# jgrss/cultionet

Measured on AMD Instinct MI355X. Metric: train_chips_per_sec, higher is better.
Workload: dtype f32

## Files before the change

cultionet_amd/_lib.py:

```python
from __future__ import annotations

import ctypes
import os
from ctypes import c_double, c_float, c_int, c_long, c_ulonglong, c_void_p

_HERE = os.path.dirname(os.path.abspath(__file__))
LIB_PATH = os.environ.get("CN_LIB_PATH") or os.path.join(_HERE, "csrc", "libcultionet_hip.so")

P = c_void_p
I, L, F, U64 = c_int, c_long, c_float, c_ulonglong

SIGNATURES = {
    "cn_version": [],
    "cn_conv_kpad": [I],
    "cn_conv_npad": [I],
    "cn_pack_weights_f32": [P, P, I, I, I, L, L, L, P],
    "cn_pack_weights_batched_f32": [P, I, P],
    "cn_conv2d_fwd_f32": [P, L, P, P, P, L, I, I, I, I, I, I, I, I, I, I, I, P],
    "cn_conv2d_bwd_data_f32": [P, L, P, P, L, I, I, I, I, I, I, I, I, I, I, I, P],
    "cn_conv2d_bwd_weight_f32": [P, L, P, L, P, I, I, I, I, I, I, I, I, I, I, P, L, P],
    "cn_conv_set_workspace": [P, P, L],
    "cn_conv_set_autotune": [I],
    "cn_conv2d_fwd_grouped_f32": [I, P, L, P, P, P, L, I, I, I, I, I, I, I, I, P, P, I, P],
    "cn_conv2d_bwd_data_grouped_f32": [I, P, L, P, P, L, I, I, I, I, I, P, P, I, P, P, I, P],
    "cn_conv2d_bwd_weight_grouped_f32": [I, P, L, P, L, P, I, I, I, I, I, I, I, I, I, I, P, L, P],
    "cn_thin_conv3x3_fwd_f32": [P, L, P, P, P, L, I, I, I, I, I, I, I, I, P, P],
    "cn_thin_conv3x3_bwd_data_f32": [P, L, P, P, L, I, I, I, I, I, I, I, I, I, P, P],
    "cn_thin_conv3x3_bwd_weight_f32": [P, L, P, L, P, I, I, I, I, I, I, I, I, P],
    "cn_conv_transpose2d_fwd_f32": [P, L, P, P, P, L, I, I, I, I, I, I, I, I, I, I, I, P],
    "cn_conv_transpose2d_bwd_data_f32": [P, L, P, P, L, I, I, I, I, I, I, I, I, I, I, I, P],
    "cn_conv_transpose2d_bwd_weight_f32": [P, L, P, L, P, I, I, I, I, I, I, I, I, I, I, P, L, P],
    "cn_channel_sum_f32": [P, L, I, I, I, P, I, P],
    "cn_bn_workspace_doubles": [I],
    "cn_bn_act_fwd_f32": [P, L, P, P, P, P, P, L, P, L, P, P, P, I, I, I, I, F, F, I, P],
    "cn_bn_act_bwd_f32": [P, L, P, L, P, P, P, P, P, L, P, P, P, P, I, I, I, I, I, I, I, P],
    "cn_bn_act_group_fwd_f32": [I, P, L, P, P, P, P, P, L, P, L, P, P, P, I, I, I, I, F, F, I, I, P],
    "cn_bn_act_group_bwd_f32": [I, P, L, P, L, P, P, P, P, P, L, P, P, P, P, I, I, I, I, I, I, P],
    "cn_layernorm_c_fwd_f32": [P, L, P, P, P, L, P, L, P, P, I, I, I, F, P],
    "cn_layernorm_c_workspace_floats": [I, I, I],
    "cn_layernorm_c_bwd_f32": [P, L, P, L, P, P, P, P, L, P, P, I, I, I, I, P, L, P],
    "cn_sca_pool_fwd_f32": [P, L, I, I, I, P, P, P, P, P, P],
    "cn_sca_pool_bwd_f32": [P, P, P, P, P, P, L, I, I, I, I, P],
    "cn_sca_mlp_fwd_f32": [P, P, P, P, P, P, P, P, P, I, I, I, P],
    "cn_sca_mlp_bwd_f32": [P, P, P, P, P, P, P, P, P, P, P, P, P, P, P, P, I, I, I, P],
    "cn_sca_apply_fwd_f32": [P, L, P, P, P, P, L, I, I, I, P],
    "cn_sca_apply_bwd_f32": [P, L, P, L, P, P, P, P, L, I, P, P, P, P, I, I, I, P],
    "cn_na2d_fwd_f32": [P, L, P, L, P, I, I, I, I, I, I, I, F, U64, P, P],
    "cn_na2d_bwd_f32": [P, L, P, L, P, P, P, L, I, I, I, I, I, I, I, F, U64, P, P],
    "cn_convt_taps_fwd_f32": [P, L, P, P, L, I, I, I, I, I, I, I, I, I, P],
    "cn_convt_taps_bwd_f32": [P, L, P, L, I, I, I, I, I, I, I, I, I, P],
    "cn_bilinear_fwd_f32": [P, L, P, L, I, I, I, I, I, I, I, I, P],
    "cn_bilinear_bwd_f32": [P, L, P, L, I, I, I, I, I, I, I, I, I, P],
    "cn_copy_f32": [P, L, P, L, I, L, I, P],
    "cn_add_f32": [P, L, P, L, P, L, I, L, P],
    "cn_fill_f32": [P, L, F, P],
    "cn_dropout_f32": [P, L, P, L, I, I, I, F, U64, P, I, I, P],
    "cn_rng_advance_u64": [P, U64, I, P],
    "cn_adaptive_maxpool_fwd_f32": [P, L, P, L, P, I, I, I, I, I, I, P],
    "cn_adaptive_maxpool_bwd_f32": [P, L, P, P, L, I, I, I, I, I, I, I, P],
    "cn_final_combine_fwd_f32": [P, P, P, P, P, P, P, I, I, F, P],
    "cn_final_combine_bwd_f32": [P, P, P, P, P, P, P, P, P, P, P, P, P, P, I, I, F, P],
    "cn_tanimoto_fwd_f32": [P, L, P, P, P, I, I, I, I, I, L, I, F, I, P, P, P, F, P, P],
    "cn_tanimoto_bwd_f32": [P, L, P, P, P, I, I, I, I, I, L, P, F, P, L, I, P],
    "cn_tanimoto_multi_fwd_f32": [I, P, I, L, I, F, I, P, P, P, P, P],
    "cn_tanimoto_multi_bwd_f32": [I, P, I, L, P, P],
    "cn_eval_metrics_f32": [P, P, P, P, P, I, F, L, P, P, P, P],
    "cn_grad_sumsq_f32": [P, L, P, P],
    "cn_adamw_step_f32": [P, P, P, P, L, F, F, F, F, F, I, F, P, F, P],
    "cn_grad_sumsq_seg_f32": [P, L, P, I, I, P, P],
    "cn_adamw_step_seg_f32": [P, P, P, P, L, P, I, I, I, F, F, F, F, F, F, P, F, P],
    "cn_pack_timeconv_f32": [P, P, I, I, I, I, I, P],
    "cn_fold_timeconv_grad_f32": [P, P, I, I, I, I, P],
    "cn_prepare_chips_f32": [P, I, P, P, P, I, I, L, F, F, F, P],
    "cn_predictions_to_u16": [P, P, P, P, I, I, I, I, I, I, I, F, P],
    "cn_bconv_packed_elems": [I, I, I],
# ... 116 lines not shown
```

cultionet_amd/csrc/cn_conv.hip:

```cpp
#include "cn_common.h"
#include "cn_conv_geom.h"
#include "cn_profile.h"

#include <cstdlib>

#define KC 8

static int cn_reduce_slices(const CnConvGeom& g, hipStream_t stream);

template <int TN, int TM>
__device__ __forceinline__ void cn_igemm_epilogue(const CnConvGeom& g, const f32x16 (&acc)[TN][TM],
                                                  const bool (&pix_ok)[TM], const int (&out_off)[TM], int co_base,
                                                  int half, int grp, int split, int b,
                                                  const float* __restrict__ bias, float* __restrict__ y) {
  const int HWout = g.Hout * g.Wout;
  const bool sliced = g.slice_stride != 0;
  float* yb = sliced ? g.part + (long)(grp * g.splits + split) * g.slice_stride + (long)b * g.Cout * HWout
                     : y + (long)b * g.ybs;
  const bool first = split == 0;
#pragma unroll
  for (int tn = 0; tn < TN; ++tn) {
#pragma unroll
    for (int r = 0; r < 16; ++r) {
      const int co = co_base + tn * 32 + (r & 3) + 8 * (r >> 2) + 4 * half;
      if (co < g.Cout) {
        const float bv = (bias != nullptr && first) ? bias[co] : 0.f;
#pragma unroll
        for (int tm = 0; tm < TM; ++tm) {
          if (pix_ok[tm]) {
            float* dst = yb + (long)co * HWout + out_off[tm];
            const float v = acc[tn][tm][r] + bv;
            if (sliced) {
              *dst = acc[tn][tm][r];
            } else if (g.atomic_out) {
              atomicAdd(dst, v);
            } else if (g.accumulate) {
              *dst += v;
            } else {
              *dst = v;
            }
          }
        }
      }
    }
  }
}

template <int WAVES_N, int TN, int NI_T>
__global__ __launch_bounds__(256) void cn_conv_igemm_kernel(const CnConvGeom g) {
  constexpr int WAVES_M = 4 / WAVES_N;
  constexpr int MT = WAVES_M * 64;
  constexpr int NT = WAVES_N * TN * 32;
  constexpr int WI = (CN_MAX_TAPS * KC * (NT / 4) + 255) / 256;
  extern __shared__ __attribute__((aligned(16))) float smem[];
  float* in_lds = smem;
  float* w_lds = smem + g.w_lds_off;
// ... 542 lines not shown
}

struct CnPlan {
  int total_tiles, max_plane, max_vplane, max_taps;
  int max_rplane, max_absdx;
  double flops;
};

static CnPlan cn_plan(CnConvGeom& g, int MT) {
  CnPlan p = {0, 0, 0, 0, 0, 0, 0.0};
  for (int c = 0; c < g.ncls; ++c) {
    CnConvClass& k = g.cls[c];
    const int Mimg = k.Hg * k.Wg;
    int rows_g = (MT + k.Wg - 2) / k.Wg + 1;
    if (rows_g > k.Hg) rows_g = k.Hg;
    k.min_dy = 0; k.min_dx = 0;
    int max_dy = 0, max_dx = 0;
    for (int t = 0; t < k.ntaps; ++t) {
      if (t == 0 || k.dy[t] < k.min_dy) k.min_dy = k.dy[t];
      if (t == 0 || k.dx[t] < k.min_dx) k.min_dx = k.dx[t];
      if (t == 0 || k.dy[t] > max_dy) max_dy = k.dy[t];
      if (t == 0 || k.dx[t] > max_dx) max_dx = k.dx[t];
    }
    const int rows = (rows_g - 1) * g.is + (max_dy - k.min_dy) + 1;
    k.pitch = (k.Wg - 1) * g.is + (max_dx - k.min_dx) + 1;
    k.plane = rows * k.pitch;
    k.vplane = (rows * g.Win + (max_dx - k.min_dx) + 4 + 3) / 4 * 4;
    k.rows = rows;
    {
      const int rpitch = (g.Win + 3) / 4 * 4 + 4;
      if ((rows + 1) * rpitch + 4 > p.max_rplane) p.max_rplane = (rows + 1) * rpitch + 4;
    }
    if (-k.min_dx > p.max_absdx) p.max_absdx = -k.min_dx;
    if (max_dx > p.max_absdx) p.max_absdx = max_dx;
    k.tiles_per_img = (Mimg + MT - 1) / MT;
    k.block_begin = p.total_tiles;
    p.total_tiles += g.B * k.tiles_per_img;
    if (k.plane > p.max_plane) p.max_plane = k.plane;
    if (k.vplane > p.max_vplane) p.max_vplane = k.vplane;
    if (k.ntaps > p.max_taps) p.max_taps = k.ntaps;
    p.flops += 2.0 * g.B * Mimg * (double)g.Cout * g.Cin * k.ntaps;
  }
  g.interleave = 0;
  if (g.ncls > 1 && g.want_interleave) {
    bool same = true;
    for (int c = 1; c < g.ncls; ++c) same = same && g.cls[c].tiles_per_img == g.cls[0].tiles_per_img;
    g.interleave = same ? 1 : 0;
  }
  return p;
}

struct CnChoice { int cfg, splits, cps; double cost; };

static double cn_launch_cost(long blocks, int cps, double mt_units, int splits, double out_elems) {
  const double F = 273.0, R = 170.0;
  const double c1 = 36.7 + 0.614 * mt_units, c2 = 30.0 + 1.19 * mt_units;
  const long full = blocks / 512, rem = blocks % 512;
  double c = full * (F + cps * c2);
  if (rem > 0) c += F + cps * (rem > 256 ? c2 : c1);
  if (splits > 1) c += R + out_elems * 4.0 * (2.0 * splits + 1.0) / 8.0e6 * (128.0 / 7.5);
  return c;
}

static thread_local float* g_conv_ws;
static thread_local long g_conv_ws_floats;

static CnChoice cn_choose(const CnConvGeom& g0, const int* mts, int ncfg, int NT, bool allow_split) {
  const int nchunks = (g0.Cin + KC - 1) / KC;
  const int ny = (g0.Cout + NT - 1) / NT;
  const int G = g0.G > 0 ? g0.G : 1;
  const double out_elems = (double)g0.B * g0.Cout * g0.Hout * g0.Wout * (g0.shared_y ? 1 : G);
  CnChoice best = {0, 1, nchunks > 0 ? nchunks : 1, 1e300};
  int forced = 0;
  {
    static const char* dbg = getenv("CN_DBG_SPLITS");
    if (dbg) forced = atoi(dbg) < 1 ? 1 : atoi(dbg);
  }
  long ws_cap = 32;
  if (g_conv_ws != nullptr) {
    const long stride = ((long)g0.B * g0.Cout * g0.Hout * g0.Wout + 3) / 4 * 4;
    ws_cap = g_conv_ws_floats / (stride * G);
  }
  int forced_cfg = -1;
  {
    static const char* dbgc = getenv("CN_DBG_CFG");
    if (dbgc) forced_cfg = atoi(dbgc);
  }
  for (int i = 0; i < ncfg; ++i) {
    if (forced_cfg >= 0 && i != (forced_cfg < ncfg ? forced_cfg : ncfg - 1)) continue;
    CnConvGeom gi = g0;
    const CnPlan p = cn_plan(gi, mts[i]);
    if (p.total_tiles <= 0) continue;
    const long base = (long)p.total_tiles * ny;
    int max_splits = (allow_split && p.max_taps > 0 && nchunks >= 4) ? nchunks / 2 : 1;
    if (max_splits > 32) max_splits = 32;
    if (max_splits > ws_cap) max_splits = ws_cap < 1 ? 1 : (int)ws_cap;
    const double taps = p.total_tiles > 0 ? p.flops / (2.0 * g0.Cout * g0.Cin * (double)mts[i] * p.total_tiles) : 9.0;
    const double chunk_units = (double)mts[i] * NT / 128.0 * (taps < 9.0 ? taps : 9.0) / 9.0;
    for (int sp = 1; sp <= max_splits; ++sp) {
      if (forced && sp != (forced > max_splits ? max_splits : forced)) continue;
      const int cps = (nchunks + sp - 1) / sp;
      const int splits = (nchunks + cps - 1) / cps;
      if (splits != sp && !forced) continue;
      const double cost = cn_launch_cost(base * splits, cps, chunk_units, splits, out_elems);
      if (cost < best.cost * (i == best.cfg ? 1.0 : 0.98)) best = {i, splits, cps, cost};
    }
  }
  return best;
}


#include <mutex>
#include <unordered_map>
namespace {
struct CnWs { float* p; long n; };
std::mutex g_ws_mu;
std::unordered_map<void*, CnWs> g_ws_by_stream;
}

extern "C" int cn_conv_set_workspace(void* stream, float* ws, long ws_floats) {
  if (ws != nullptr && ((reinterpret_cast<uintptr_t>(ws) & 15) || ws_floats < 0)) return CN_ERR_ARG;
  std::lock_guard<std::mutex> lk(g_ws_mu);
  if (ws == nullptr) g_ws_by_stream.erase(stream);
  else g_ws_by_stream[stream] = {ws, ws_floats};
  return CN_OK;
}

static void cn_bind_ws(void* stream) {
  std::lock_guard<std::mutex> lk(g_ws_mu);
  auto it = g_ws_by_stream.find(stream);
  if (it == g_ws_by_stream.end()) { g_conv_ws = nullptr; g_conv_ws_floats = 0; }
  else { g_conv_ws = it->second.p; g_conv_ws_floats = it->second.n; }
}

struct CnReduceArgs {
  const float* part;
  long slice_stride;
  int nsum;
  int ngrp;
  float* y[CN_MAX_GROUPS];
  const float* bias[CN_MAX_GROUPS * CN_MAX_GROUPS];
  int nbias;
  long ybs;
  int B, Cout, HW, accumulate;
};

__global__ __launch_bounds__(256) void cn_conv_reduce_kernel(const CnReduceArgs a) {
  const long n = (long)a.Cout * a.HW;
  const int b = blockIdx.y, gi = blockIdx.z;
  const float* p0 = a.part + (long)gi * a.nsum * a.slice_stride + (long)b * n;
  float* yb = a.y[gi] + (long)b * a.ybs;
  for (long i = (blockIdx.x * 256L + threadIdx.x) * 4; i < n; i += (long)gridDim.x * 1024) {
    if (i + 3 < n && (n & 3) == 0 && (a.ybs & 3) == 0 && (reinterpret_cast<uintptr_t>(yb) & 15) == 0) {
      f32x4 s = *reinterpret_cast<const f32x4*>(p0 + i);
      for (int k = 1; k < a.nsum; ++k) s += *reinterpret_cast<const f32x4*>(p0 + (long)k * a.slice_stride + i);
#pragma unroll
      for (int e = 0; e < 4; ++e) {
        const int c = (int)((i + e) / a.HW);
// ... 168 lines not shown
    __syncthreads();
#pragma unroll
    for (int k = 0; k < NA; ++k) *reinterpret_cast<f32x4*>(a_lds + (tid + k * 256) * 4) = ra[k];
#pragma unroll
    for (int k = 0; k < NB; ++k)
      if (tid + k * 256 < KC1 * MT / 4) *reinterpret_cast<f32x4*>(b_lds + (tid + k * 256) * 4) = rb[k];
    __syncthreads();
    if (ch + 1 < nchunks) CN_G1_PREFETCH((ch + 1) * KC1);
    const float* ap = a_lds + half * NT + wn * 32 + l31;
    const float* bp = b_lds + half * MT + l31;
#pragma unroll
    for (int k2 = 0; k2 < KC1 / 2; ++k2) {
      const float av = ap[k2 * 2 * NT];
#pragma unroll
      for (int tm = 0; tm < TM; ++tm)
        acc[tm] = __builtin_amdgcn_mfma_f32_32x32x2f32(av, bp[k2 * 2 * MT + tm * 32], acc[tm], 0, 0, 0);
    }
  }
#undef CN_G1_PREFETCH
  float* yb = y + (long)b * g.ybs;
#pragma unroll
  for (int r = 0; r < 16; ++r) {
    const int co = n0 + wn * 32 + (r & 3) + 8 * (r >> 2) + 4 * half;
    if (co < g.Cout) {
      const float bv = bias != nullptr ? bias[co] : 0.f;
#pragma unroll
      for (int tm = 0; tm < TM; ++tm) {
        const int p = p0 + tm * 32 + l31;
        if (p < g.HW) {
          float* dst = yb + (long)co * g.HW + p;
          const float v = acc[tm][r] + bv;
          *dst = g.accumulate ? *dst + v : v;
        }
      }
    }
  }
}

static int cn_conv1x1_launch(const float* x, long xbs, const float* wp, const float* bias, float* y, long ybs, int B,
                             int Cin, int HW, int Cout, int accumulate, hipStream_t stream) {
  if ((HW & 3) || (xbs & 3) || (reinterpret_cast<uintptr_t>(x) & 15)) return CN_ERR_ARG;
  CnGemm1x1 g = {};
  g.B = B; g.Cin = Cin; g.Cout = Cout; g.HW = HW; g.xbs = xbs; g.ybs = ybs; g.accumulate = accumulate;
  g.Kpad = cn_conv_kpad(Cin);
  g.Npad = cn_conv_npad(Cout);
  if (cn_pick_nt(Cout) != 128) return CN_ERR_ARG;
  g.grid_y = (Cout + 127) / 128;
  const long t160 = (long)B * ((HW + 159) / 160) * g.grid_y, t128 = (long)B * ((HW + 127) / 128) * g.grid_y;
  const bool use160 = ((t160 + 511) / 512) * 160 <= ((t128 + 511) / 512) * 128;
  const long blocks = use160 ? t160 : t128;
  if (blocks < 256) return CN_ERR_ARG;
  g.tiles_per_img = use160 ? (HW + 159) / 160 : (HW + 127) / 128;
  g.grid_x = B * g.tiles_per_img;
  const double flops = 2.0 * B * HW * (double)Cout * Cin;
  cn_prof_name("cn_conv1x1_kernel<%d>", use160 ? 5 : 4);
  cn_prof_desc("gemm1x1<%d> B%d %d->%d HW%d grid%dx%d", use160 ? 5 : 4, B, Cin, Cout, HW, g.grid_x, g.grid_y);
  cn_prof_before(stream);
  if (use160)
    CN_LAUNCH((cn_conv1x1_kernel<5>), dim3(cn_xcd_grid(blocks)), dim3(256), 0, stream, x, wp, bias, y, g);
  else
    CN_LAUNCH((cn_conv1x1_kernel<4>), dim3(cn_xcd_grid(blocks)), dim3(256), 0, stream, x, wp, bias, y, g);
  cn_prof_after(stream, 0, flops);
  return cn_check_launch();
}

#include <functional>
static int g_autotune = 0;
static std::unordered_map<uint64_t, CnChoice> g_tuned;
static std::mutex g_tune_mu;

extern "C" int cn_conv_set_autotune(int on) {
  std::lock_guard<std::mutex> lk(g_tune_mu);
  g_autotune = on ? 1 : 0;
  if (!on) g_tuned.clear();
  return CN_OK;
}

static uint64_t cn_tune_key(const CnConvGeom& g, bool vec, int nt, bool allow_split) {
  uint64_t h = 1469598103934665603ull;
  auto mix = [&](long v) { h = (h ^ (uint64_t)v) * 1099511628211ull; };
  mix(g.B); mix(g.Cin); mix(g.Hin); mix(g.Win); mix(g.Cout); mix(g.Hout); mix(g.Wout); mix(g.is); mix(g.os);
  mix(g.ncls); mix(g.G); mix(g.shared_y); mix(vec); mix(nt); mix(allow_split); mix(g_conv_ws != nullptr);
  for (int c = 0; c < g.ncls; ++c) {
    const CnConvClass& k = g.cls[c];
    mix(k.Hg); mix(k.Wg); mix(k.ntaps); mix(k.grp);
    for (int t = 0; t < k.ntaps; ++t) { mix(k.dy[t]); mix(k.dx[t]); }
  }
  return h;
}

static CnChoice cn_autotune(const CnConvGeom& g, const int* mts, int ncfg, int nt, bool allow_split,
                            const CnChoice& model, const std::function<int(const CnChoice&, CnConvGeom&)>& run,
                            hipStream_t stream) {
  static const int split_set[] = {1, 2, 3, 4, 6, 8, 12, 16, 24, 32};
  const int nchunks = (g.Cin + KC - 1) / KC;
  const int ny = (g.Cout + nt - 1) / nt;
  long ws_cap = 32;
  if (g_conv_ws != nullptr) {
    const long stride = ((long)g.B * g.Cout * g.Hout * g.Wout + 3) / 4 * 4;
    ws_cap = g_conv_ws_floats / (stride * (g.G > 0 ? g.G : 1));
  }
  hipEvent_t e0, e1;
  if (hipEventCreate(&e0) != hipSuccess || hipEventCreate(&e1) != hipSuccess) return model;
  CnChoice best = model;
  float best_ms = 1e30f;
  for (int i = 0; i < ncfg; ++i) {
    CnConvGeom gi = g;
    const CnPlan p = cn_plan(gi, mts[i]);
    if (p.total_tiles <= 0) continue;
    int max_splits = (allow_split && p.max_taps > 0 && nchunks >= 4) ? nchunks / 2 : 1;
    if (max_splits > 32) max_splits = 32;
    if (max_splits > ws_cap) max_splits = ws_cap < 1 ? 1 : (int)ws_cap;
    for (int sp : split_set) {
      if (sp > max_splits) break;
      const int cps = (nchunks + sp - 1) / sp;
      const int splits = (nchunks + cps - 1) / cps;
      if (splits != sp) continue;
      if ((long)p.total_tiles * ny * splits > 8192) continue;
      const CnChoice c = {i, splits, cps, 0.0};
      float ms = 0.f;
      bool ok = true;
      for (int rep = 0; rep < 2 && ok; ++rep) {
        CnConvGeom gg = g;
        ok = hipEventRecord(e0, stream) == hipSuccess && run(c, gg) == CN_OK &&
             hipEventRecord(e1, stream) == hipSuccess && hipEventSynchronize(e1) == hipSuccess &&
             hipEventElapsedTime(&ms, e0, e1) == hipSuccess;
      }
      if (ok && ms < best_ms) { best_ms = ms; best = c; }
    }
  }
  (void)hipEventDestroy(e0);
  (void)hipEventDestroy(e1);
  return best;
}

int cn_conv_igemm_launch(CnConvGeom& g, hipStream_t stream) {
  if (g.ncls < 1 || g.ncls > CN_MAX_CLASSES || g.B <= 0 || g.G < 1) return g.B <= 0 ? CN_OK : CN_ERR_ARG;
  g.splits = 1;
  const float* x = g.gx[0]; const float* wp = g.gwp[0]; const float* bias = g.gbias[0]; float* y = g.gy[0];
  g.Kpad = cn_conv_kpad(g.Cin);
  g.Npad = cn_conv_npad(g.Cout);
  const int nt = cn_pick_nt(g.Cout);
  const bool dense_out = g.ybs == (long)g.Cout * g.Hout * g.Wout;
  const bool ws_fits = g_conv_ws != nullptr &&
                       (((long)g.B * g.Cout * g.Hout * g.Wout + 3) / 4 * 4) * g.G * 32 <= g_conv_ws_floats;
  const bool allow_split = dense_out || g.accumulate || ws_fits;
  if (g.G > 1 && g.shared_y && !allow_split) return CN_ERR_ARG;
  const int hw4 = (int)(((long)g.Hin * g.Win) % 4);
  g.odd_planes = (hw4 == 1 && !(g.is > 1 && (long)g.Hin * g.Win > 4096)) ? 1 : 0;
  bool vec = (hw4 == 0 || g.odd_planes) && (g.xbs % 4 == 0);
  if (g.is > 1 && (long)g.Hin * g.Win > 4096) vec = false;
  if ((long)g.Cin * g.Hin * g.Win * 4 >= (1L << 31) || (long)CN_MAX_TAPS * cn_conv_kpad(g.Cin) * g.Npad * 4 >= (1L << 31))
    return CN_ERR_ARG;
  for (int i = 0; i < g.G; ++i) vec = vec && ((reinterpret_cast<uintptr_t>(g.gx[i]) & 15) == 0);
  if (vec) {
    CnConvGeom t = g;
    vec = cn_plan(t, 256).max_vplane <= 4 * 1024;
  }
  static const int mts128[3] = {128, 96, 160};
  static const int mts128d[1] = {128};
  static const int mts256[1] = {256};
  const int* mts = nt == 128 ? (vec ? mts128 : mts128d) : mts256;
  const int ncfg = (nt == 128 && vec) ? 3 : 1;
  auto run = [&](const CnChoice& c, CnConvGeom& gg) -> int {
    if (nt == 128) {
      if (vec) {
        switch (c.cfg) {
          case 1: return cn_launch_vec_cfg<4, 1, 3>(x, wp, bias, y, gg, c.splits, c.cps, stream);
          case 2: return cn_launch_vec_cfg<4, 1, 5>(x, wp, bias, y, gg, c.splits, c.cps, stream);
          default: return cn_launch_vec_cfg<2, 2, 2>(x, wp, bias, y, gg, c.splits, c.cps, stream);
        }
      }
      return cn_launch_dword_cfg<2, 2>(x, wp, bias, y, gg, c.splits, c.cps, stream);
    }
    int rc;
    if (nt == 64) {
      if (vec) return cn_launch_vec_cfg<1, 2, 2>(x, wp, bias, y, gg, c.splits, c.cps, stream);
      rc = cn_launch_dword_cfg<1, 2>(x, wp, bias, y, gg, c.splits, c.cps, stream);
    } else {
      if (vec) return cn_launch_vec_cfg<1, 1, 2>(x, wp, bias, y, gg, c.splits, c.cps, stream);
      rc = cn_launch_dword_cfg<1, 1>(x, wp, bias, y, gg, c.splits, c.cps, stream);
    }
    if (rc == CN_ERR_LDS) {
      CnConvGeom g2 = gg;
      rc = cn_launch_dword_cfg<2, 2>(x, wp, bias, y, g2, c.splits, c.cps, stream);
    }
    return rc;
  };
  CnChoice c = cn_choose(g, mts, ncfg, nt, allow_split);
  if (g_autotune) {
    std::lock_guard<std::mutex> lk(g_tune_mu);
    const uint64_t key = cn_tune_key(g, vec, nt, allow_split);
    auto it = g_tuned.find(key);
    if (it != g_tuned.end()) {
      c = it->second;
    } else if (!g.accumulate && !cn_prof_on()) {
      c = cn_autotune(g, mts, ncfg, nt, allow_split, c, run, stream);
      g_tuned.emplace(key, c);
    }
  }
  return run(c, g);
}

static inline int floordiv(int a, int b) { return (a >= 0) ? a / b : -((-a + b - 1) / b); }

static int cn_set_groups(CnConvGeom& g, int G, const float* const* xs, const float* const* wps,
                         const float* const* biases, float* const* ys) {
  if (G < 1 || G > CN_MAX_GROUPS) return CN_ERR_ARG;
  g.G = G;
  int same = 0;
  for (int i = 0; i < G; ++i) {
    g.gx[i] = xs[i]; g.gwp[i] = wps[i]; g.gbias[i] = biases ? biases[i] : nullptr; g.gy[i] = ys[i];
    if (ys[i] == ys[0]) ++same;
  }
  if (same != G && same != 1) return CN_ERR_ARG;
  for (int i = 1; i < G && same == 1; ++i)
    for (int j = 1; j < i; ++j)
      if (ys[i] == ys[j]) return CN_ERR_ARG;
  g.shared_y = (G > 1 && same == G) ? 1 : 0;
  g.has_bias = 0;
  for (int i = 0; i < G; ++i) g.has_bias |= g.gbias[i] != nullptr;
  return CN_OK;
}

static int cn_gather_conv_g(int G, const float* const* xs, long xbs, const float* const* wps,
                            const float* const* biases, float* const* ys, long ybs, int B, int Cin, int Hin,
                            int Win, int Cout, int Hout, int Wout, int KH, int KW, int stride, const int* pads,
                            const int* dils, int accumulate, hipStream_t stream) {
  if (KH * KW > CN_MAX_TAPS || stride < 1) return CN_ERR_ARG;
  if (Hout <= 0 || Wout <= 0) return CN_OK;
  if (G == 1 && KH == 1 && KW == 1 && stride == 1 && pads[0] == 0 && Hout == Hin && Wout == Win) {
    const int r1 = cn_conv1x1_launch(xs[0], xbs, wps[0], biases ? biases[0] : nullptr, ys[0], ybs, B, Cin, Hin * Win,
                                     Cout, accumulate, stream);
    if (r1 != CN_ERR_ARG) return r1;
  }
  CnConvGeom g = {};
  const int rc = cn_set_groups(g, G, xs, wps, biases, ys);
  if (rc != CN_OK) return rc;
  g.B = B; g.Cin = Cin; g.Hin = Hin; g.Win = Win; g.Cout = Cout; g.Hout = Hout; g.Wout = Wout;
  g.xbs = xbs; g.ybs = ybs; g.is = stride; g.os = 1;
  g.ncls = G;
  for (int i = 0; i < G; ++i) {
    if (dils[i] < 1) return CN_ERR_ARG;
    CnConvClass& k = g.cls[i];
    k.grp = i;
    k.Hg = Hout; k.Wg = Wout; k.oy0 = 0; k.ox0 = 0;
    k.ntaps = KH * KW;
    for (int ky = 0; ky < KH; ++ky)
      for (int kx = 0; kx < KW; ++kx) {
        const int t = ky * KW + kx;
        k.dy[t] = ky * dils[i] - pads[i]; k.dx[t] = kx * dils[i] - pads[i]; k.wt[t] = t;
      }
// ... 103 lines not shown
  if (G < 1 || G > CN_MAX_GROUPS) return CN_ERR_ARG;
  if (stride < 1) return CN_ERR_ARG;
  const int Hout = (Hin + 2 * pads[0] - dils[0] * (KH - 1) - 1) / stride + 1;
  const int Wout = (Win + 2 * pads[0] - dils[0] * (KW - 1) - 1) / stride + 1;
  for (int i = 1; i < G; ++i)
    if ((Hin + 2 * pads[i] - dils[i] * (KH - 1) - 1) / stride + 1 != Hout ||
        (Win + 2 * pads[i] - dils[i] * (KW - 1) - 1) / stride + 1 != Wout)
      return CN_ERR_ARG;
  return cn_gather_conv_g(G, xs, xbs, wps, biases, ys, ybs, B, Cin, Hin, Win, Cout, Hout, Wout, KH, KW, stride,
                          pads, dils, accumulate, (hipStream_t)stream);
}

extern "C" int cn_conv2d_bwd_data_grouped_f32(int G, const float* const* dys, long dybs, const float* const* wps_t,
                                              float* const* dxs, long dxbs, int B, int Cin, int Hin, int Win,
                                              int Cout, const int* khs, const int* kws, int stride, const int* pads,
                                              const int* dils, int accumulate, void* stream) {
  cn_bind_ws(stream);
  if (G < 1 || G > CN_MAX_GROUPS) return CN_ERR_ARG;
  if (stride < 1) return CN_ERR_ARG;
  const int Hout = (Hin + 2 * pads[0] - dils[0] * (khs[0] - 1) - 1) / stride + 1;
  const int Wout = (Win + 2 * pads[0] - dils[0] * (kws[0] - 1) - 1) / stride + 1;
  for (int i = 1; i < G; ++i)
    if ((Hin + 2 * pads[i] - dils[i] * (khs[i] - 1) - 1) / stride + 1 != Hout ||
        (Win + 2 * pads[i] - dils[i] * (kws[i] - 1) - 1) / stride + 1 != Wout)
      return CN_ERR_ARG;
  return cn_scatter_conv_g(G, dys, dybs, wps_t, nullptr, dxs, dxbs, B, Cout, Hout, Wout, Cin, Hin, Win, khs, kws,
                           stride, pads, dils, accumulate, (hipStream_t)stream);
}

extern "C" int cn_conv_transpose2d_fwd_f32(const float* x, long xbs, const float* wp, const float* bias,
                                           float* y, long ybs, int B, int Cin, int Hin, int Win, int Cout,
                                           int KH, int KW, int stride, int pad, int out_pad, int accumulate,
                                           void* stream) {
  cn_bind_ws(stream);
  if (out_pad < 0 || (out_pad > 0 && out_pad >= stride)) return CN_ERR_ARG;
  const int Hout = (Hin - 1) * stride - 2 * pad + KH + out_pad;
  const int Wout = (Win - 1) * stride - 2 * pad + KW + out_pad;
  return cn_scatter_conv(x, xbs, wp, bias, y, ybs, B, Cin, Hin, Win, Cout, Hout, Wout, KH, KW, stride, pad, 1,
                         accumulate, (hipStream_t)stream);
}

extern "C" int cn_conv_transpose2d_bwd_data_f32(const float* dy, long dybs, const float* wp_t, float* dx,
                                                long dxbs, int B, int Cin, int Hin, int Win, int Cout, int KH,
                                                int KW, int stride, int pad, int out_pad, int accumulate,
                                                void* stream) {
  cn_bind_ws(stream);
  if (out_pad < 0 || (out_pad > 0 && out_pad >= stride)) return CN_ERR_ARG;
  const int Hout = (Hin - 1) * stride - 2 * pad + KH + out_pad;
  const int Wout = (Win - 1) * stride - 2 * pad + KW + out_pad;
  return cn_gather_conv(dy, dybs, wp_t, nullptr, dx, dxbs, B, Cout, Hout, Wout, Cin, Hin, Win, KH, KW, stride, pad,
                        1, accumulate, (hipStream_t)stream);
}

__global__ void cn_pack_timeconv_kernel(const float* __restrict__ w, float* __restrict__ wp, int Cout, int Cin,
                                        int Tin, int k, int transposed, int Kpad, int Npad) {
  const int Tout = Tin - k + 1;
  const int Kd = transposed ? Cout * Tout : Cin * Tin;
  const int Nd = transposed ? Cin * Tin : Cout * Tout;
  const long total = (long)Kpad * Npad;
  for (long i = blockIdx.x * (long)blockDim.x + threadIdx.x; i < total; i += (long)gridDim.x * blockDim.x) {
    const int n = (int)(i % Npad), kk = (int)(i / Npad);
    float v = 0.f;
    if (kk < Kd && n < Nd) {
      const int in_idx = transposed ? n : kk, out_idx = transposed ? kk : n;
      const int ci = in_idx / Tin, t = in_idx - ci * Tin;
      const int co = out_idx / Tout, tp = out_idx - co * Tout;
      const int dt = t - tp;
      if (dt >= 0 && dt < k) v = w[((long)co * Cin + ci) * k + dt];
    }
    wp[i] = v;
  }
}

extern "C" int cn_pack_timeconv_f32(const float* w, float* wp, int Cout, int Cin, int Tin, int k, int transposed,
                                    void* stream) {
  const int Tout = Tin - k + 1;
  if (Tout < 1) return CN_ERR_ARG;
  const int Kd = transposed ? Cout * Tout : Cin * Tin, Nd = transposed ? Cin * Tin : Cout * Tout;
  const int Kpad = cn_conv_kpad(Kd), Npad = cn_conv_npad(Nd);
  const long total = (long)Kpad * Npad;
  CN_LAUNCH(cn_pack_timeconv_kernel, dim3((unsigned)((total + 255) / 256)), dim3(256), 0,
                     (hipStream_t)stream, w, wp, Cout, Cin, Tin, k, transposed, Kpad, Npad);
  return cn_check_launch();
}

__global__ void cn_fold_timeconv_kernel(const float* __restrict__ dwexp, float* __restrict__ dw, int Cout, int Cin,
                                        int Tin, int k) {
  const int Tout = Tin - k + 1;
  const int i = blockIdx.x * blockDim.x + threadIdx.x;
  if (i >= Cout * Cin * k) return;
  const int dt = i % k, ci = (i / k) % Cin, co = i / (k * Cin);
  float s = 0.f;
  for (int tp = 0; tp < Tout; ++tp) s += dwexp[(long)(co * Tout + tp) * (Cin * Tin) + ci * Tin + tp + dt];
  dw[i] += s;
}

extern "C" int cn_fold_timeconv_grad_f32(const float* dwexp, float* dw, int Cout, int Cin, int Tin, int k,
                                         void* stream) {
  const int n = Cout * Cin * k;
  CN_LAUNCH(cn_fold_timeconv_kernel, dim3((n + 63) / 64), dim3(64), 0, (hipStream_t)stream, dwexp, dw, Cout,
                     Cin, Tin, k);
  return cn_check_launch();
}
```

cultionet_amd/csrc/cn_optim.hip:

```cpp
#include "cn_common.h"

__global__ __launch_bounds__(256) void cn_sumsq_kernel(const float* __restrict__ g, long n, double* __restrict__ out) {
  __shared__ double scratch[4];
  double s = 0.0;
  for (long i = blockIdx.x * 256L + threadIdx.x; i < n; i += (long)gridDim.x * 256) {
    const float v = g[i];
    s += (double)v * v;
  }
  s = cn_block_sum<double, 256>(s, scratch);
  if (threadIdx.x == 0) atomicAdd(out, s);
}

extern "C" int cn_grad_sumsq_f32(const float* g, long n, double* out, void* stream_) {
  hipStream_t stream = (hipStream_t)stream_;
  if (hipMemsetAsync(out, 0, sizeof(double), stream) != hipSuccess) return CN_ERR_LAUNCH;
  if (n <= 0) return CN_OK;
  long bx = (n + 2047) / 2048;
  if (bx > 1024) bx = 1024;
  CN_LAUNCH(cn_sumsq_kernel, dim3((unsigned)bx), dim3(256), 0, stream, g, n, out);
  return cn_check_launch();
}

__global__ __launch_bounds__(256) void cn_adamw_kernel(float* __restrict__ p, const float* __restrict__ g,
                                                      float* __restrict__ m, float* __restrict__ v, long n, float lr,
// ... 79 lines not shown
  if (nseg < 0 || nchunks < 0 || n < 0) return CN_ERR_ARG;
  if (hipMemsetAsync(out, 0, sizeof(double), stream) != hipSuccess) return CN_ERR_LAUNCH;
  if (nseg == 0 || nchunks == 0) return CN_OK;
  CN_LAUNCH(cn_sumsq_seg_kernel, dim3((unsigned)cn_seg_grid(nchunks, 1024)), dim3(256), 0, stream, g, n,
            (const CnSeg*)segs, nseg, nchunks, out);
  return cn_check_launch();
}

__global__ __launch_bounds__(256) void cn_adamw_seg_kernel(float* __restrict__ p, const float* __restrict__ g,
                                                          float* __restrict__ m, float* __restrict__ v, long n,
                                                          const CnSeg* __restrict__ segs, int nseg, int nchunks,
                                                          int step_add, float lr, float b1, float b2, float eps, float wd,
                                                          float grad_scale, const double* sumsq, float max_norm) {
  float gs = grad_scale;
  if (sumsq != nullptr) {
    const float norm = (float)sqrt(*sumsq) * grad_scale;
    const float coef = max_norm / (norm + 1e-6f);
    gs *= fminf(coef, 1.0f);
  }
  for (int c = blockIdx.x; c < nchunks; c += gridDim.x) {
    const CnSeg sg = segs[cn_seg_find(segs, nseg, c)];
    const long lo = sg.off + (long)(c - sg.chunk0) * CN_SEG_CHUNK;
    long hi = sg.off + sg.len;
    if (hi > lo + CN_SEG_CHUNK) hi = lo + CN_SEG_CHUNK;
    if (hi > n) hi = n;
    const double t = (double)sg.step + step_add;
    const float bc1 = (float)(1.0 - pow((double)b1, t));
    const float bc2_sqrt = (float)sqrt(1.0 - pow((double)b2, t));
    const float step = lr / bc1;
    for (long i = lo + threadIdx.x; i < hi; i += 256) {
      const float gi = g[i] * gs;
      float pi = p[i] * (1.f - lr * wd);
      const float mi = b1 * m[i] + (1.f - b1) * gi;
      const float vi = b2 * v[i] + (1.f - b2) * gi * gi;
      pi -= step * mi / (sqrtf(vi) / bc2_sqrt + eps);
      p[i] = pi;
      m[i] = mi;
      v[i] = vi;
    }
  }
}

extern "C" int cn_adamw_step_seg_f32(float* p, const float* g, float* m, float* v, long n, const void* segs, int nseg,
                                     int nchunks, int step_add, float lr, float beta1, float beta2, float eps, float weight_decay,
                                     float grad_scale, const double* sumsq, float max_norm, void* stream) {
  if (nseg < 0 || nchunks < 0 || n < 0) return CN_ERR_ARG;
  if (nseg == 0 || nchunks == 0) return CN_OK;
  CN_LAUNCH(cn_adamw_seg_kernel, dim3((unsigned)cn_seg_grid(nchunks, 2048)), dim3(256), 0, (hipStream_t)stream, p, g,
            m, v, n, (const CnSeg*)segs, nseg, nchunks, step_add, lr, beta1, beta2, eps, weight_decay, grad_scale, sumsq,
            max_norm);
  return cn_check_launch();
}

extern "C" int cn_version() { return 101; }
```

include/cultionet_hip.h:

```cpp
#ifndef CULTIONET_HIP_H
#define CULTIONET_HIP_H

#ifdef __cplusplus
extern "C" {
#endif

#define CN_OK 0
#define CN_ERR_ARG (-1)
#define CN_ERR_LAUNCH (-2)
#define CN_ERR_LDS (-3)

int cn_version(void);

int cn_conv_kpad(int k_in);
int cn_conv_npad(int n_out);
int cn_pack_weights_f32(const float* w, float* wp, int T, int K, int N, long sk, long sn, long st, void* stream);
int cn_pack_weights_batched_f32(const void* descs, int n, void* stream);

int cn_conv2d_fwd_f32(const float* x, long xbs, const float* wp, const float* bias , float* y, long ybs,
                      int B, int Cin, int Hin, int Win, int Cout, int KH, int KW, int stride, int pad, int dil,
                      int accumulate, void* stream);
int cn_conv2d_bwd_data_f32(const float* dy, long dybs, const float* wp_t, float* dx, long dxbs, int B, int Cin,
                           int Hin, int Win, int Cout, int KH, int KW, int stride, int pad, int dil, int accumulate,
                           void* stream);
int cn_conv2d_bwd_weight_f32(const float* x, long xbs, const float* dy, long dybs, float* dw, int B, int Cin, int Hin,
                             int Win, int Cout, int KH, int KW, int stride, int pad, int dil, float* ws,
                             long ws_floats, void* stream);

int cn_pack_timeconv_f32(const float* w, float* wp, int Cout, int Cin, int Tin, int k, int transposed, void* stream);
int cn_fold_timeconv_grad_f32(const float* dwexp, float* dw, int Cout, int Cin, int Tin, int k, void* stream);

int cn_conv_transpose2d_fwd_f32(const float* x, long xbs, const float* wp, const float* bias, float* y, long ybs,
                                int B, int Cin, int Hin, int Win, int Cout, int KH, int KW, int stride, int pad,
                                int out_pad, int accumulate, void* stream);
int cn_conv_transpose2d_bwd_data_f32(const float* dy, long dybs, const float* wp_t, float* dx, long dxbs, int B,
                                     int Cin, int Hin, int Win, int Cout, int KH, int KW, int stride, int pad,
                                     int out_pad, int accumulate, void* stream);
int cn_conv_transpose2d_bwd_weight_f32(const float* x, long xbs, const float* dy, long dybs, float* dw, int B, int Cin,
                                       int Hin, int Win, int Cout, int KH, int KW, int stride, int pad, int out_pad,
                                       float* ws, long ws_floats, void* stream);

int cn_conv_set_workspace(void* stream, float* ws, long ws_floats);

int cn_conv_set_autotune(int on);

int cn_conv2d_fwd_grouped_f32(int G, const float* const* xs, long xbs, const float* const* wps,
                              const float* const* biases , float* const* ys, long ybs, int B, int Cin,
                              int Hin, int Win, int Cout, int KH, int KW, int stride, const int* pads,
                              const int* dils, int accumulate, void* stream);
int cn_conv2d_bwd_data_grouped_f32(int G, const float* const* dys, long dybs, const float* const* wps_t,
                                   float* const* dxs, long dxbs, int B, int Cin, int Hin, int Win, int Cout,
                                   const int* khs, const int* kws ,
                                   int stride, const int* pads, const int* dils, int accumulate, void* stream);

int cn_conv2d_bwd_weight_grouped_f32(int G, const float* const* xs, long xbs, const float* const* dys, long dybs,
                                     float* const* dws, int B, int Cin, int Hin, int Win, int Cout, int KH, int KW,
                                     int stride, int pad, int dil, float* ws, long ws_floats, void* stream);

int cn_thin_conv3x3_fwd_f32(const float* x, long xbs, const float* const* ws, const float* const* biases ,
                            float* y, long ybs, int B, int Cin, int H, int W, int nsets, int cout_per_set,
                            int grouped, int dil, float* wpack , void* stream);
int cn_thin_conv3x3_bwd_data_f32(const float* dy, long dybs, const float* const* ws, float* dx, long dxbs, int B,
                                 int Cin, int H, int W, int nsets, int cout_per_set, int grouped, int dil,
                                 int accumulate, float* wpack , void* stream);
int cn_thin_conv3x3_bwd_weight_f32(const float* x, long xbs, const float* dy, long dybs, float* const* dws, int B,
                                   int Cin, int H, int W, int nsets, int cout_per_set, int grouped, int dil,
                                   void* stream);

int cn_channel_sum_f32(const float* x, long xbs, int B, int C, int L, float* out, int accumulate, void* stream);

int cn_bn_workspace_doubles(int C);
int cn_bn_act_fwd_f32(const float* x, long xbs, const float* gamma, const float* beta, float* running_mean,
                      float* running_var, const float* res , long rbs, float* y, long ybs, float* mean,
                      float* rstd, double* ws, int B, int C, int L, int training, float momentum, float eps, int act,
                      void* stream);
int cn_bn_act_bwd_f32(const float* x, long xbs, const float* dy, long dybs, const float* mean, const float* rstd,
                      const float* gamma, const float* beta, float* dx , long dxbs, float* dgamma,
                      float* dbeta, float* coef, double* ws, int B, int C, int L, int training, int act,
                      int accumulate_dx, int accumulate_params, void* stream);

int cn_bn_act_group_fwd_f32(int G, const float* const* xs, long xbs, const float* const* gammas,
                            const float* const* betas, float* const* running_means, float* const* running_vars,
                            const float* res , long rbs, float* const* ys, long ybs, float* const* means,
                            float* const* rstds, double* ws, int B, int C, int L, int training, float momentum,
                            float eps, int act, int sum_outputs, void* stream);
int cn_bn_act_group_bwd_f32(int G, const float* const* xs, long xbs, const float* const* dys, long dybs,
                            const float* const* means, const float* const* rstds, const float* const* gammas,
                            const float* const* betas, float* const* dxs, long dxbs, const int* accumulate_dx,
                            float* const* dgammas, float* const* dbetas, double* ws, int B, int C, int L,
                            int training, int act, int accumulate_params, void* stream);

int cn_layernorm_c_fwd_f32(const float* x, long xbs, const float* w, const float* b, const float* res ,
                           long rbs, float* y, long ybs, float* mu, float* rstd, int B, int C, int L, float eps,
                           void* stream);
int cn_layernorm_c_bwd_f32(const float* x, long xbs, const float* dy, long dybs, const float* w, const float* mu,
                           const float* rstd, float* dx, long dxbs, float* dw, float* db, int B, int C, int L,
                           int accumulate_dx, float* ws, long ws_floats, void* stream);
// ... 241 lines not shown
```

Before: 389.8.

## Add narrower N-tile configs to implicit-GEMM conv selection and plan query

Extends the implicit-GEMM conv tile candidate set with narrower output-channel tiles (64 and 32 wide) for both the vec and dword paths. The cost model scales their per-chunk cost by a stage-share factor, and they are considered when wider tiles need split-K. The autotuner now takes the min over repeated timings instead of the last one, and can dump its measurements. A plan-query entry point is also added. The aim is better occupancy for small-Cout or split-heavy layers, at the cost of more kernel instantiations and a model that may pick worse tiles.

```diff
diff --git a/cultionet_amd/_lib.py b/cultionet_amd/_lib.py
--- a/cultionet_amd/_lib.py
+++ b/cultionet_amd/_lib.py
@@ -21,6 +21,7 @@
     "cn_conv2d_bwd_weight_f32": [P, L, P, L, P, I, I, I, I, I, I, I, I, I, I, P, L, P],
     "cn_conv_set_workspace": [P, P, L],
     "cn_conv_set_autotune": [I],
+    "cn_conv_plan_query": [I, I, I, I, I, I, I, I, I, I, I, I, I, I, P, P],
     "cn_conv2d_fwd_grouped_f32": [I, P, L, P, P, P, L, I, I, I, I, I, I, I, I, P, P, I, P],
     "cn_conv2d_bwd_data_grouped_f32": [I, P, L, P, P, L, I, I, I, I, I, P, P, I, P, P, I, P],
     "cn_conv2d_bwd_weight_grouped_f32": [I, P, L, P, L, P, I, I, I, I, I, I, I, I, I, I, P, L, P],
diff --git a/cultionet_amd/csrc/cn_conv.hip b/cultionet_amd/csrc/cn_conv.hip
--- a/cultionet_amd/csrc/cn_conv.hip
+++ b/cultionet_amd/csrc/cn_conv.hip
@@ -2,6 +2,7 @@
 #include "cn_conv_geom.h"
 #include "cn_profile.h"
 
+#include <cstdio>
 #include <cstdlib>
 
 #define KC 8
@@ -650,6 +651,8 @@
 
 struct CnChoice { int cfg, splits, cps; double cost; };
 
+struct CnTile { int nt, mt; };
+
 static double cn_launch_cost(long blocks, int cps, double mt_units, int splits, double out_elems) {
   const double F = 273.0, R = 170.0;
   const double c1 = 36.7 + 0.614 * mt_units, c2 = 30.0 + 1.19 * mt_units;
@@ -663,9 +666,15 @@
 static thread_local float* g_conv_ws;
 static thread_local long g_conv_ws_floats;
 
-static CnChoice cn_choose(const CnConvGeom& g0, const int* mts, int ncfg, int NT, bool allow_split) {
+static thread_local int* g_plan_out;
+
+#define CN_STAGE_SHARE (1.0 / 3.0)
+#define CN_NARROW_GAIN 0.98
+
+static CnChoice cn_choose(const CnConvGeom& g0, const CnTile* tiles, int ncfg, int n0, bool narrow_by_model,
+                          bool allow_split) {
   const int nchunks = (g0.Cin + KC - 1) / KC;
-  const int ny = (g0.Cout + NT - 1) / NT;
+  const int NT = tiles[0].nt;
   const int G = g0.G > 0 ? g0.G : 1;
   const double out_elems = (double)g0.B * g0.Cout * g0.Hout * g0.Wout * (g0.shared_y ? 1 : G);
   CnChoice best = {0, 1, nchunks > 0 ? nchunks : 1, 1e300};
@@ -684,24 +693,46 @@
     static const char* dbgc = getenv("CN_DBG_CFG");
     if (dbgc) forced_cfg = atoi(dbgc);
   }
-  for (int i = 0; i < ncfg; ++i) {
-    if (forced_cfg >= 0 && i != (forced_cfg < ncfg ? forced_cfg : ncfg - 1)) continue;
+  int forced_nt = 0;
+  {
+    static const char* dbgn = getenv("CN_DBG_NT");
+    if (dbgn) forced_nt = atoi(dbgn);
+  }
+  if (forced_nt > 0) {
+    int t = forced_nt < 32 ? 32 : forced_nt;
+    for (;; t *= 2) {
+      bool found = false;
+      for (int i = 0; i < ncfg; ++i) found = found || tiles[i].nt == t;
+      if (found || t >= NT) break;
+    }
+    forced_nt = t < NT ? t : NT;
+  }
+  int sel[16], nsel = 0;
+  for (int i = 0; i < ncfg && nsel < 16; ++i)
+    if (forced_nt > 0 ? tiles[i].nt == forced_nt : (i < n0 || forced_cfg >= 0 || narrow_by_model)) sel[nsel++] = i;
+  for (int s = 0; s < nsel; ++s) {
+    const int i = sel[s];
+    if (forced_cfg >= 0 && s != (forced_cfg < nsel ? forced_cfg : nsel - 1)) continue;
+    if (i >= n0 && forced_nt <= 0 && forced_cfg < 0 && best.splits == 1) break;
+    const int ny = (g0.Cout + tiles[i].nt - 1) / tiles[i].nt;
     CnConvGeom gi = g0;
-    const CnPlan p = cn_plan(gi, mts[i]);
+    const CnPlan p = cn_plan(gi, tiles[i].mt);
     if (p.total_tiles <= 0) continue;
     const long base = (long)p.total_tiles * ny;
     int max_splits = (allow_split && p.max_taps > 0 && nchunks >= 4) ? nchunks / 2 : 1;
     if (max_splits > 32) max_splits = 32;
     if (max_splits > ws_cap) max_splits = ws_cap < 1 ? 1 : (int)ws_cap;
-    const double taps = p.total_tiles > 0 ? p.flops / (2.0 * g0.Cout * g0.Cin * (double)mts[i] * p.total_tiles) : 9.0;
-    const double chunk_units = (double)mts[i] * NT / 128.0 * (taps < 9.0 ? taps : 9.0) / 9.0;
+    const double taps =
+        p.total_tiles > 0 ? p.flops / (2.0 * g0.Cout * g0.Cin * (double)tiles[i].mt * p.total_tiles) : 9.0;
+    double chunk_units = (double)tiles[i].mt * NT / 128.0 * (taps < 9.0 ? taps : 9.0) / 9.0;
+    if (tiles[i].nt != NT) chunk_units *= CN_STAGE_SHARE + (1.0 - CN_STAGE_SHARE) * tiles[i].nt / NT;
     for (int sp = 1; sp <= max_splits; ++sp) {
       if (forced && sp != (forced > max_splits ? max_splits : forced)) continue;
       const int cps = (nchunks + sp - 1) / sp;
       const int splits = (nchunks + cps - 1) / cps;
       if (splits != sp && !forced) continue;
       const double cost = cn_launch_cost(base * splits, cps, chunk_units, splits, out_elems);
-      if (cost < best.cost * (i == best.cfg ? 1.0 : 0.98)) best = {i, splits, cps, cost};
+      if (cost < best.cost * (i == best.cfg ? 1.0 : (i >= n0 ? CN_NARROW_GAIN : 0.98))) best = {i, splits, cps, cost};
     }
   }
   return best;
@@ -976,6 +1007,11 @@
   if (blocks < 256) return CN_ERR_ARG;
   g.tiles_per_img = use160 ? (HW + 159) / 160 : (HW + 127) / 128;
   g.grid_x = B * g.tiles_per_img;
+  if (g_plan_out != nullptr) {
+    const int plan[6] = {128, use160 ? 160 : 128, -1, 1, (Cin + KC1 - 1) / KC1, (int)blocks};
+    for (int i = 0; i < 6; ++i) g_plan_out[i] = plan[i];
+    return CN_OK;
+  }
   const double flops = 2.0 * B * HW * (double)Cout * Cin;
   cn_prof_name("cn_conv1x1_kernel<%d>", use160 ? 5 : 4);
   cn_prof_desc("gemm1x1<%d> B%d %d->%d HW%d grid%dx%d", use160 ? 5 : 4, B, Cin, Cout, HW, g.grid_x, g.grid_y);
@@ -1000,11 +1036,11 @@
   return CN_OK;
 }
 
-static uint64_t cn_tune_key(const CnConvGeom& g, bool vec, int nt, bool allow_split) {
+static uint64_t cn_tune_key(const CnConvGeom& g, bool vec, int nt, int ncfg, bool allow_split) {
   uint64_t h = 1469598103934665603ull;
   auto mix = [&](long v) { h = (h ^ (uint64_t)v) * 1099511628211ull; };
   mix(g.B); mix(g.Cin); mix(g.Hin); mix(g.Win); mix(g.Cout); mix(g.Hout); mix(g.Wout); mix(g.is); mix(g.os);
-  mix(g.ncls); mix(g.G); mix(g.shared_y); mix(vec); mix(nt); mix(allow_split); mix(g_conv_ws != nullptr);
+  mix(g.ncls); mix(g.G); mix(g.shared_y); mix(vec); mix(nt); mix(ncfg); mix(allow_split); mix(g_conv_ws != nullptr);
   for (int c = 0; c < g.ncls; ++c) {
     const CnConvClass& k = g.cls[c];
     mix(k.Hg); mix(k.Wg); mix(k.ntaps); mix(k.grp);
@@ -1013,12 +1049,14 @@
   return h;
 }
 
-static CnChoice cn_autotune(const CnConvGeom& g, const int* mts, int ncfg, int nt, bool allow_split,
-                            const CnChoice& model, const std::function<int(const CnChoice&, CnConvGeom&)>& run,
-                            hipStream_t stream) {
+static CnChoice cn_autotune(const CnConvGeom& g, const CnTile* tiles, int ncfg, bool allow_split, const CnChoice& model,
+                            const std::function<int(const CnChoice&, CnConvGeom&)>& run, hipStream_t stream) {
   static const int split_set[] = {1, 2, 3, 4, 6, 8, 12, 16, 24, 32};
+  static FILE* dump = [] {
+    const char* path = getenv("CN_TUNE_DUMP");
+    return path ? fopen(path, "a") : (FILE*)nullptr;
+  }();
   const int nchunks = (g.Cin + KC - 1) / KC;
-  const int ny = (g.Cout + nt - 1) / nt;
   long ws_cap = 32;
   if (g_conv_ws != nullptr) {
     const long stride = ((long)g.B * g.Cout * g.Hout * g.Wout + 3) / 4 * 4;
@@ -1030,8 +1068,9 @@
   float best_ms = 1e30f;
   for (int i = 0; i < ncfg; ++i) {
     CnConvGeom gi = g;
-    const CnPlan p = cn_plan(gi, mts[i]);
+    const CnPlan p = cn_plan(gi, tiles[i].mt);
     if (p.total_tiles <= 0) continue;
+    const int ny = (g.Cout + tiles[i].nt - 1) / tiles[i].nt;
     int max_splits = (allow_split && p.max_taps > 0 && nchunks >= 4) ? nchunks / 2 : 1;
     if (max_splits > 32) max_splits = 32;
     if (max_splits > ws_cap) max_splits = ws_cap < 1 ? 1 : (int)ws_cap;
@@ -1042,21 +1081,31 @@
       if (splits != sp) continue;
       if ((long)p.total_tiles * ny * splits > 8192) continue;
       const CnChoice c = {i, splits, cps, 0.0};
-      float ms = 0.f;
+      float ms = 1e30f;
       bool ok = true;
-      for (int rep = 0; rep < 2 && ok; ++rep) {
+      for (int rep = 0; rep < 4 && ok; ++rep) {
         CnConvGeom gg = g;
+        float t = 0.f;
         ok = hipEventRecord(e0, stream) == hipSuccess && run(c, gg) == CN_OK &&
              hipEventRecord(e1, stream) == hipSuccess && hipEventSynchronize(e1) == hipSuccess &&
-             hipEventElapsedTime(&ms, e0, e1) == hipSuccess;
-      }
+             hipEventElapsedTime(&t, e0, e1) == hipSuccess;
+        if (ok && rep > 0 && t < ms) ms = t;
+      }
+      if (ok && dump)
+        fprintf(dump, "G%d B%d %d->%d %dx%d->%dx%d taps%d cls%d is%d os%d\t%d\t%d\t%d\t%d\t%ld\t%.1f\t%s\n", g.G, g.B,
+                g.Cin, g.Cout, g.Hin, g.Win, g.Hout, g.Wout, p.max_taps, g.ncls, g.is, g.os, tiles[i].nt, tiles[i].mt,
+                splits, cps, (long)p.total_tiles * ny * splits, ms * 1e3,
+                (i == model.cfg && splits == model.splits) ? "model" : "");
       if (ok && ms < best_ms) { best_ms = ms; best = c; }
     }
   }
+  if (dump) fflush(dump);
   (void)hipEventDestroy(e0);
   (void)hipEventDestroy(e1);
   return best;
 }
+
+static constexpr int cn_tile_id(int nt, int mt) { return nt * 1000 + mt; }
 
 int cn_conv_igemm_launch(CnConvGeom& g, hipStream_t stream) {
   if (g.ncls < 1 || g.ncls > CN_MAX_CLASSES || g.B <= 0 || g.G < 1) return g.B <= 0 ? CN_OK : CN_ERR_ARG;
@@ -1081,47 +1130,58 @@
     CnConvGeom t = g;
     vec = cn_plan(t, 256).max_vplane <= 4 * 1024;
   }
-  static const int mts128[3] = {128, 96, 160};
-  static const int mts128d[1] = {128};
-  static const int mts256[1] = {256};
-  const int* mts = nt == 128 ? (vec ? mts128 : mts128d) : mts256;
-  const int ncfg = (nt == 128 && vec) ? 3 : 1;
+  static const CnTile tv128[6] = {{128, 128}, {128, 96}, {128, 160}, {64, 128}, {64, 192}, {32, 128}};
+  static const CnTile td128[2] = {{128, 128}, {64, 128}};
+  static const CnTile t64[2] = {{64, 256}, {32, 256}};
+  static const CnTile t32[1] = {{32, 256}};
+  const CnTile* tiles = nt == 128 ? (vec ? tv128 : td128) : (nt == 64 ? t64 : t32);
+  const int ncfg = nt == 128 ? (vec ? 6 : 2) : (nt == 64 ? 2 : 1);
+  const int n0 = (nt == 128 && vec) ? 3 : 1;
+  const bool narrow_by_model = nt == 128;
   auto run = [&](const CnChoice& c, CnConvGeom& gg) -> int {
-    if (nt == 128) {
-      if (vec) {
-        switch (c.cfg) {
-          case 1: return cn_launch_vec_cfg<4, 1, 3>(x, wp, bias, y, gg, c.splits, c.cps, stream);
-          case 2: return cn_launch_vec_cfg<4, 1, 5>(x, wp, bias, y, gg, c.splits, c.cps, stream);
-          default: return cn_launch_vec_cfg<2, 2, 2>(x, wp, bias, y, gg, c.splits, c.cps, stream);
-        }
-      }
-      return cn_launch_dword_cfg<2, 2>(x, wp, bias, y, gg, c.splits, c.cps, stream);
-    }
-    int rc;
-    if (nt == 64) {
-      if (vec) return cn_launch_vec_cfg<1, 2, 2>(x, wp, bias, y, gg, c.splits, c.cps, stream);
-      rc = cn_launch_dword_cfg<1, 2>(x, wp, bias, y, gg, c.splits, c.cps, stream);
-    } else {
-      if (vec) return cn_launch_vec_cfg<1, 1, 2>(x, wp, bias, y, gg, c.splits, c.cps, stream);
-      rc = cn_launch_dword_cfg<1, 1>(x, wp, bias, y, gg, c.splits, c.cps, stream);
-    }
+    const int id = cn_tile_id(tiles[c.cfg].nt, tiles[c.cfg].mt);
+    if (vec) {
+      switch (id) {
+        case cn_tile_id(128, 128): return cn_launch_vec_cfg<2, 2, 2>(x, wp, bias, y, gg, c.splits, c.cps, stream);
+        case cn_tile_id(128, 96): return cn_launch_vec_cfg<4, 1, 3>(x, wp, bias, y, gg, c.splits, c.cps, stream);
+        case cn_tile_id(128, 160): return cn_launch_vec_cfg<4, 1, 5>(x, wp, bias, y, gg, c.splits, c.cps, stream);
+        case cn_tile_id(64, 128): return cn_launch_vec_cfg<2, 1, 2>(x, wp, bias, y, gg, c.splits, c.cps, stream);
+        case cn_tile_id(64, 192): return cn_launch_vec_cfg<2, 1, 3>(x, wp, bias, y, gg, c.splits, c.cps, stream);
+        case cn_tile_id(32, 128): return cn_launch_vec_cfg<1, 1, 1>(x, wp, bias, y, gg, c.splits, c.cps, stream);
+        case cn_tile_id(64, 256): return cn_launch_vec_cfg<1, 2, 2>(x, wp, bias, y, gg, c.splits, c.cps, stream);
+        default: return cn_launch_vec_cfg<1, 1, 2>(x, wp, bias, y, gg, c.splits, c.cps, stream);
+      }
+    }
+    if (id == cn_tile_id(128, 128)) return cn_launch_dword_cfg<2, 2>(x, wp, bias, y, gg, c.splits, c.cps, stream);
+    if (id == cn_tile_id(64, 128)) return cn_launch_dword_cfg<2, 1>(x, wp, bias, y, gg, c.splits, c.cps, stream);
+    int rc = id == cn_tile_id(64, 256) ? cn_launch_dword_cfg<1, 2>(x, wp, bias, y, gg, c.splits, c.cps, stream)
+                                       : cn_launch_dword_cfg<1, 1>(x, wp, bias, y, gg, c.splits, c.cps, stream);
     if (rc == CN_ERR_LDS) {
       CnConvGeom g2 = gg;
       rc = cn_launch_dword_cfg<2, 2>(x, wp, bias, y, g2, c.splits, c.cps, stream);
     }
     return rc;
   };
-  CnChoice c = cn_choose(g, mts, ncfg, nt, allow_split);
+  CnChoice c = cn_choose(g, tiles, ncfg, n0, narrow_by_model, allow_split);
   if (g_autotune) {
     std::lock_guard<std::mutex> lk(g_tune_mu);
-    const uint64_t key = cn_tune_key(g, vec, nt, allow_split);
+    const uint64_t key = cn_tune_key(g, vec, nt, ncfg, allow_split);
     auto it = g_tuned.find(key);
     if (it != g_tuned.end()) {
       c = it->second;
-    } else if (!g.accumulate && !cn_prof_on()) {
-      c = cn_autotune(g, mts, ncfg, nt, allow_split, c, run, stream);
+    } else if (!g.accumulate && !cn_prof_on() && g_plan_out == nullptr) {
+      c = cn_autotune(g, tiles, ncfg, allow_split, c, run, stream);
       g_tuned.emplace(key, c);
     }
+  }
+  if (g_plan_out != nullptr) {
+    CnConvGeom t = g;
+    const CnPlan p = cn_plan(t, tiles[c.cfg].mt);
+    const int ny = (g.Cout + tiles[c.cfg].nt - 1) / tiles[c.cfg].nt;
+    const int plan[6] = {tiles[c.cfg].nt, tiles[c.cfg].mt, c.cfg, c.splits, c.cps,
+                         (int)((long)p.total_tiles * ny * c.splits)};
+    for (int i = 0; i < 6; ++i) g_plan_out[i] = plan[i];
+    return CN_OK;
   }
   return run(c, g);
 }
@@ -1331,6 +1391,47 @@
                         1, accumulate, (hipStream_t)stream);
 }
 
+extern "C" int cn_conv_plan_query(int kind, int G, int shared_y, int B, int Cin, int Hin, int Win, int Cout, int KH,
+                                  int KW, int stride, int pad, int dil, int out_pad, void* stream, int* plan) {
+  if (plan == nullptr || kind < 0 || kind > 3 || G < 1 || G > CN_MAX_GROUPS || (kind >= 2 && G != 1) || stride < 1 ||
+      B < 1)
+    return CN_ERR_ARG;
+  for (int i = 0; i < 6; ++i) plan[i] = 0;
+  const float* in[CN_MAX_GROUPS];
+  const float* wp[CN_MAX_GROUPS];
+  float* out[CN_MAX_GROUPS];
+  int pads[CN_MAX_GROUPS], dils[CN_MAX_GROUPS], khs[CN_MAX_GROUPS], kws[CN_MAX_GROUPS];
+  for (int i = 0; i < CN_MAX_GROUPS; ++i) {
+    in[i] = reinterpret_cast<const float*>((uintptr_t)4096 * (1 + i));
+    wp[i] = reinterpret_cast<const float*>((uintptr_t)4096 * (9 + i));
+    out[i] = reinterpret_cast<float*>((uintptr_t)4096 * (17 + (shared_y ? 0 : i)));
+    pads[i] = pad; dils[i] = dil; khs[i] = KH; kws[i] = KW;
+  }
+  hipStream_t st = (hipStream_t)stream;
+  cn_bind_ws(stream);
+  g_plan_out = plan;
+  int rc = CN_ERR_ARG;
+  if (kind < 2) {
+    const int Hout = (Hin + 2 * pad - dil * (KH - 1) - 1) / stride + 1;
+    const int Wout = (Win + 2 * pad - dil * (KW - 1) - 1) / stride + 1;
+    const long isz = (long)Cin * Hin * Win, osz = (long)Cout * Hout * Wout;
+    rc = kind == 0 ? cn_gather_conv_g(G, in, isz, wp, nullptr, out, osz, B, Cin, Hin, Win, Cout, Hout, Wout, KH, KW,
+                                      stride, pads, dils, 0, st)
+                   : cn_scatter_conv_g(G, in, osz, wp, nullptr, out, isz, B, Cout, Hout, Wout, Cin, Hin, Win, khs, kws,
+                                       stride, pads, dils, 0, st);
+  } else if (out_pad >= 0 && (out_pad == 0 || out_pad < stride)) {
+    const int Hout = (Hin - 1) * stride - 2 * pad + KH + out_pad;
+    const int Wout = (Win - 1) * stride - 2 * pad + KW + out_pad;
+    const long isz = (long)Cin * Hin * Win, osz = (long)Cout * Hout * Wout;
+    rc = kind == 2 ? cn_scatter_conv(in[0], isz, wp[0], nullptr, out[0], osz, B, Cin, Hin, Win, Cout, Hout, Wout, KH,
+                                     KW, stride, pad, 1, 0, st)
+                   : cn_gather_conv(in[0], osz, wp[0], nullptr, out[0], isz, B, Cout, Hout, Wout, Cin, Hin, Win, KH, KW,
+                                    stride, pad, 1, 0, st);
+  }
+  g_plan_out = nullptr;
+  return rc;
+}
+
 __global__ void cn_pack_timeconv_kernel(const float* __restrict__ w, float* __restrict__ wp, int Cout, int Cin,
                                         int Tin, int k, int transposed, int Kpad, int Npad) {
   const int Tout = Tin - k + 1;
diff --git a/cultionet_amd/csrc/cn_optim.hip b/cultionet_amd/csrc/cn_optim.hip
--- a/cultionet_amd/csrc/cn_optim.hip
+++ b/cultionet_amd/csrc/cn_optim.hip
@@ -155,4 +155,4 @@
   return cn_check_launch();
 }
 
-extern "C" int cn_version() { return 101; }
+extern "C" int cn_version() { return 102; }
diff --git a/include/cultionet_hip.h b/include/cultionet_hip.h
--- a/include/cultionet_hip.h
+++ b/include/cultionet_hip.h
@@ -43,6 +43,9 @@
 int cn_conv_set_workspace(void* stream, float* ws, long ws_floats);
 
 int cn_conv_set_autotune(int on);
+
+int cn_conv_plan_query(int kind, int G, int shared_y, int B, int Cin, int Hin, int Win, int Cout, int KH, int KW,
+                       int stride, int pad, int dil, int out_pad, void* stream, int* plan);
 
 int cn_conv2d_fwd_grouped_f32(int G, const float* const* xs, long xbs, const float* const* wps,
                               const float* const* biases , float* const* ys, long ybs, int B, int Cin,
```

Result: no change. 390.9 (median of 2 runs) (+0.3%).
